# nerfstudio-project/gsplat

Measured on AMD Instinct MI355X. Metric: Mpixels/s fwd+bwd @1M Gaussians/1080p, higher is better.
Workload: dtype f32; 1 GPU; c3: 1M synthetic Gaussians, 1x1920x1080, SH deg 3, 16x16 tiles, fwd+bwd; gaussians_per_gpu=1000000, cameras_per_gpu=1, packed=False, parallelism=single

## Files before the change

gsplat_amd/csrc/projection.hip:

```cpp
#include "projmath.hpp"

namespace gsx {

struct ProjArgs {
    const float *means, *covars, *quats, *scales, *opacities, *viewmats, *Ks;
    uint32_t B, C, N, width, height;
    float eps2d, near_plane, far_plane, radius_clip;
    int camera_model;
    int calc_compensations;
    int32_t *radii;
    float *means2d, *depths, *conics, *compensations;
    int32_t *visible;
    const int64_t *row_offsets;
    int64_t nnz;
    int64_t *batch_ids, *camera_ids, *gaussian_ids;
    int32_t *indptr;
};

struct ProjOut {
    bool ok;
    int rx, ry;
    float mx, my, depth, ca, cb, cc, comp;
};

__device__ __forceinline__ void load_world_covar(const ProjArgs &a, uint32_t b, uint32_t g, float *S)
{
    if (a.covars) {
        const float *c = a.covars + ((size_t)b * a.N + g) * 6;
        S[0] = c[0]; S[1] = c[1]; S[2] = c[2];
        S[3] = c[1]; S[4] = c[3]; S[5] = c[4];
        S[6] = c[2]; S[7] = c[4]; S[8] = c[5];
    } else {
        const float *q = a.quats + ((size_t)b * a.N + g) * 4;
        const float *s = a.scales + ((size_t)b * a.N + g) * 3;
        float qn[4], Rq[9];
        quat_normalize(q, qn);
        quat_to_rotmat(qn, Rq);
        quat_scale_to_covar(Rq, s, false, S);
    }
}

__device__ __forceinline__ ProjOut project_one(const ProjArgs &a, uint32_t b, uint32_t c, uint32_t g, const float *p,
                                               float *world, bool *have_world)
{
    ProjOut o;
    o.ok = false;
    o.rx = o.ry = 0;
    o.mx = o.my = o.depth = o.ca = o.cb = o.cc = o.comp = 0.0f;
    const Cam cam  = load_cam(a.viewmats + ((size_t)b * a.C + c) * 16, a.Ks + ((size_t)b * a.C + c) * 9);
    float pc[3];
#pragma unroll
    for (int i = 0; i < 3; ++i) pc[i] = cam.R[3 * i] * p[0] + cam.R[3 * i + 1] * p[1] + cam.R[3 * i + 2] * p[2] + cam.t[i];
    if (pc[2] < a.near_plane || pc[2] > a.far_plane) return o;

    float RS[9], Sc[9];
    if (!*have_world) {
        load_world_covar(a, b, g, world);
        *have_world = true;
    }
    const float *S = world;
    mm3(cam.R, S, RS);
    mm3_nt(RS, cam.R, Sc);

    const Proj2D pr = project_camera(a.camera_model, cam, a.width, a.height, pc, Sc);
    const float det_orig = pr.a * pr.d - pr.b * pr.b;
    const float ca = pr.a + a.eps2d, cd = pr.d + a.eps2d;
    const float det_blur = ca * cd - pr.b * pr.b;
    if (det_blur <= 0.0f) return o;
    const float comp = sqrtf(fmaxf(kMinCompensation * kMinCompensation, det_orig / det_blur));

    float extend = kGaussianExtend;
    if (a.opacities) {
        float opacity = a.opacities[(size_t)b * a.N + g];
        if (a.calc_compensations) opacity *= comp;
        if (opacity < kAlphaThreshold) return o;
        extend = fminf(kGaussianExtend, sqrtf(2.0f * det_logf(opacity * 255.0f)));
    }
    const float rx = ceilf(extend * sqrtf(ca)), ry = ceilf(extend * sqrtf(cd));
    if (rx <= a.radius_clip && ry <= a.radius_clip) return o;
    if (pr.mx + rx <= 0.0f || pr.mx - rx >= (float)a.width || pr.my + ry <= 0.0f || pr.my - ry >= (float)a.height) return o;

    const float inv_det = 1.0f / det_blur;
    o.ok = true;
    o.rx = (int)rx; o.ry = (int)ry;
    o.mx = pr.mx; o.my = pr.my; o.depth = pc[2];
    o.ca = cd * inv_det; o.cb = -pr.b * inv_det; o.cc = ca * inv_det;
    o.comp = comp;
    return o;
}

__device__ __forceinline__ ProjOut project_one(const ProjArgs &a, uint32_t b, uint32_t c, uint32_t g)
{
    float world[9];
    bool have_world = false;
    return project_one(a, b, c, g, a.means + ((size_t)b * a.N + g) * 3, world, &have_world);
}

__global__ void __launch_bounds__(256) project_fwd_kernel(const ProjArgs a)
{
    const int64_t idx   = (int64_t)blockIdx.x * blockDim.x + threadIdx.x;
    const int64_t count = (int64_t)a.B * a.C * a.N;
    if (idx >= count) return;
    const uint32_t g = (uint32_t)(idx % a.N), c = (uint32_t)((idx / a.N) % a.C), b = (uint32_t)(idx / ((int64_t)a.N * a.C));
    const ProjOut o  = project_one(a, b, c, g);
    a.radii[2 * idx]       = o.rx;
    a.radii[2 * idx + 1]   = o.ry;
    a.means2d[2 * idx]     = o.mx;
    a.means2d[2 * idx + 1] = o.my;
    a.depths[idx]          = o.depth;
    a.conics[3 * idx]      = o.ca;
    a.conics[3 * idx + 1]  = o.cb;
    a.conics[3 * idx + 2]  = o.cc;
    if (a.compensations) a.compensations[idx] = o.comp;
}

__global__ void __launch_bounds__(256) project_fwd_gaussian_major_kernel(const ProjArgs a)
{
    const int64_t bg = (int64_t)blockIdx.x * blockDim.x + threadIdx.x;
    if (bg >= (int64_t)a.B * a.N) return;
    const uint32_t b = (uint32_t)(bg / a.N), g = (uint32_t)(bg % a.N);
    const float *pm = a.means + (size_t)bg * 3;
    const float p[3] = {pm[0], pm[1], pm[2]};
    float world[9];
    bool have_world = false;
    for (uint32_t c = 0; c < a.C; ++c) {
        const ProjOut o   = project_one(a, b, c, g, p, world, &have_world);
        const int64_t idx = ((int64_t)b * a.C + c) * a.N + g;
        a.radii[2 * idx]       = o.rx;
        a.radii[2 * idx + 1]   = o.ry;
        a.means2d[2 * idx]     = o.mx;
        a.means2d[2 * idx + 1] = o.my;
        a.depths[idx]          = o.depth;
        a.conics[3 * idx]      = o.ca;
        a.conics[3 * idx + 1]  = o.cb;
        a.conics[3 * idx + 2]  = o.cc;
        if (a.compensations) a.compensations[idx] = o.comp;
    }
}

__global__ void __launch_bounds__(256) project_count_kernel(const ProjArgs a)
{
    const int64_t idx   = (int64_t)blockIdx.x * blockDim.x + threadIdx.x;
    const int64_t count = (int64_t)a.B * a.C * a.N;
    if (idx >= count) return;
    const uint32_t g = (uint32_t)(idx % a.N), c = (uint32_t)((idx / a.N) % a.C), b = (uint32_t)(idx / ((int64_t)a.N * a.C));
    a.visible[idx]   = project_one(a, b, c, g).ok ? 1 : 0;
}

__global__ void __launch_bounds__(256) project_write_kernel(const ProjArgs a)
{
    const int64_t idx   = (int64_t)blockIdx.x * blockDim.x + threadIdx.x;
    const int64_t count = (int64_t)a.B * a.C * a.N;
    if (idx > count) return;
    if (idx % a.N == 0) {
        const int64_t img = idx / a.N;
        a.indptr[img]     = (int32_t)(idx == 0 ? 0 : a.row_offsets[idx - 1]);
    }
    if (idx == count) return;
    const int64_t row  = idx == 0 ? 0 : a.row_offsets[idx - 1];
    const int64_t next = a.row_offsets[idx];
    if (next == row) return;
    const uint32_t g = (uint32_t)(idx % a.N), c = (uint32_t)((idx / a.N) % a.C), b = (uint32_t)(idx / ((int64_t)a.N * a.C));
    const ProjOut o  = project_one(a, b, c, g);
    a.batch_ids[row]       = b;
    a.camera_ids[row]      = c;
    a.gaussian_ids[row]    = g;
    a.radii[2 * row]       = o.rx;
    a.radii[2 * row + 1]   = o.ry;
    a.means2d[2 * row]     = o.mx;
    a.means2d[2 * row + 1] = o.my;
    a.depths[row]          = o.depth;
    a.conics[3 * row]      = o.ca;
    a.conics[3 * row + 1]  = o.cb;
    a.conics[3 * row + 2]  = o.cc;
    if (a.compensations) a.compensations[row] = o.comp;
}

struct PackedBlocks {
    int32_t *block_counts;
    const int32_t *block_offsets;
};

__global__ void __launch_bounds__(256) project_count_blocks_kernel(const ProjArgs a, PackedBlocks pb)
{
    __shared__ int32_t s_n[4];
    const int64_t idx   = (int64_t)blockIdx.x * blockDim.x + threadIdx.x;
    const int64_t count = (int64_t)a.B * a.C * a.N;
    bool ok = false;
    if (idx < count) {
        const uint32_t g = (uint32_t)(idx % a.N), c = (uint32_t)((idx / a.N) % a.C), b = (uint32_t)(idx / ((int64_t)a.N * a.C));
        ok = project_one(a, b, c, g).ok;
    }
    const uint64_t m = __builtin_amdgcn_ballot_w64(ok);
    if ((threadIdx.x & 63u) == 0) s_n[threadIdx.x >> 6] = (int32_t)__popcll(m);
    __syncthreads();
    if (threadIdx.x == 0) pb.block_counts[blockIdx.x] = s_n[0] + s_n[1] + s_n[2] + s_n[3];
}

__global__ void __launch_bounds__(1024) packed_block_scan_kernel(const int32_t *counts, uint32_t n_blocks, int32_t *offsets,
                                                                int64_t *nnz_device, int64_t *nnz_host)
{
    __shared__ int64_t s_part[16];
    const int64_t total = block_scan_i32_1024(counts, offsets, n_blocks, s_part, nullptr);
    if (threadIdx.x == 0) {
        if (nnz_device) *nnz_device = total;
        if (nnz_host) {
            __threadfence_system();
            *nnz_host = total;
        }
    }
}

__global__ void __launch_bounds__(256) project_write_blocks_kernel(const ProjArgs a, PackedBlocks pb)
{
    __shared__ int32_t s_n[4];
    const int64_t idx   = (int64_t)blockIdx.x * blockDim.x + threadIdx.x;
    const int64_t count = (int64_t)a.B * a.C * a.N;
    const uint32_t lane = threadIdx.x & 63u, wave = threadIdx.x >> 6;
    uint32_t b = 0, c = 0, g = 0;
    ProjOut o;
    o.ok = false;
    if (idx < count) {
        g = (uint32_t)(idx % a.N); c = (uint32_t)((idx / a.N) % a.C); b = (uint32_t)(idx / ((int64_t)a.N * a.C));
        o = project_one(a, b, c, g);
    }
    const uint64_t m = __builtin_amdgcn_ballot_w64(o.ok);
    if (lane == 0) s_n[wave] = (int32_t)__popcll(m);
    __syncthreads();
    int32_t before = pb.block_offsets[blockIdx.x];
    for (uint32_t w = 0; w < wave; ++w) before += s_n[w];
    const int64_t row = (int64_t)before + (int64_t)__popcll(m & ((lane == 0) ? 0ull : (~0ull >> (64 - lane))));
    if (idx <= count && idx % a.N == 0) a.indptr[idx / a.N] = (int32_t)row;
    if (!o.ok) return;
    a.batch_ids[row]       = b;
    a.camera_ids[row]      = c;
    a.gaussian_ids[row]    = g;
    a.radii[2 * row]       = o.rx;
    a.radii[2 * row + 1]   = o.ry;
    a.means2d[2 * row]     = o.mx;
    a.means2d[2 * row + 1] = o.my;
    a.depths[row]          = o.depth;
    a.conics[3 * row]      = o.ca;
    a.conics[3 * row + 1]  = o.cb;
    a.conics[3 * row + 2]  = o.cc;
    if (a.compensations) a.compensations[row] = o.comp;
}

struct ProjBwdArgs {
    const float *means, *covars, *quats, *scales, *viewmats, *Ks;
    uint32_t B, C, N, width, height;
    float eps2d;
    int camera_model;
    const int32_t *radii;
    const float *conics, *compensations;
    const float *v_means2d, *v_depths, *v_conics, *v_compensations;
    uint32_t m2_stride, con_stride;
    int64_t nnz;
    const int64_t *batch_ids, *camera_ids, *gaussian_ids;
    const int32_t *row_map;
    int rows_out;
    float *v_means, *v_covars, *v_quats, *v_scales, *v_viewmats;
    const float *v_view_opacities;
    uint32_t opac_stride;
    float *v_opacities;
};

__device__ __forceinline__ void pair_vjp(const ProjBwdArgs &a, const Cam &cam, const float *p, const float *S,
                                         int64_t row, float *v_p, float *v_S, float *v_R, float *v_t, bool want_pose)
{
    const float ca = a.conics[3 * row], cb = a.conics[3 * row + 1], cc = a.conics[3 * row + 2];
    const float *vcon = a.v_conics + (size_t)a.con_stride * row;
    const float va = vcon[0], vb = 0.5f * vcon[1], vc = vcon[2];
    const float t00 = va * ca + vb * cb, t01 = va * cb + vb * cc;
    const float t10 = vb * ca + vc * cb, t11 = vb * cb + vc * cc;
    float g00 = -(ca * t00 + cb * t10);
    float g01 = -(ca * t01 + cb * t11);
    float g11 = -(cb * t01 + cc * t11);
    if (a.v_compensations) {
        const float comp = a.compensations[row], v_comp = a.v_compensations[row];
        const float detP = ca * cc - cb * cb;
        const float vsq  = v_comp * 0.5f / (comp + 1e-6f);
        const float omc  = 1.0f - comp * comp;
        g00 += vsq * (omc * ca - a.eps2d * detP);
        g01 += vsq * (omc * cb);
        g11 += vsq * (omc * cc - a.eps2d * detP);
    }
    float pc[3];
#pragma unroll
    for (int i = 0; i < 3; ++i) pc[i] = cam.R[3 * i] * p[0] + cam.R[3 * i + 1] * p[1] + cam.R[3 * i + 2] * p[2] + cam.t[i];
    float RS[9], Sc[9];
    mm3(cam.R, S, RS);
    mm3_nt(RS, cam.R, Sc);

    float v_pc[3] = {0.f, 0.f, 0.f}, v_Sc[9];
#pragma unroll
    for (int i = 0; i < 9; ++i) v_Sc[i] = 0.0f;
    const float *vm2 = a.v_means2d + (size_t)a.m2_stride * row;
    project_camera_vjp(a.camera_model, cam, a.width, a.height, pc, Sc, g00, g01, g11, vm2[0], vm2[1], v_pc, v_Sc);
    if (a.v_depths) v_pc[2] += a.v_depths[row];

#pragma unroll
    for (int j = 0; j < 3; ++j) v_p[j] += cam.R[j] * v_pc[0] + cam.R[3 + j] * v_pc[1] + cam.R[6 + j] * v_pc[2];
    float tmp[9], add[9];
    mm3_tn(cam.R, v_Sc, tmp);
    mm3(tmp, cam.R, add);
#pragma unroll
    for (int i = 0; i < 9; ++i) v_S[i] += add[i];
    if (want_pose) {
        float A1[9], A2[9];
        mm3(v_Sc, RS, A1);
        float v_ScT[9];
#pragma unroll
        for (int i = 0; i < 3; ++i)
#pragma unroll
            for (int j = 0; j < 3; ++j) v_ScT[3 * i + j] = v_Sc[3 * j + i];
        mm3(v_ScT, RS, A2);
#pragma unroll
        for (int i = 0; i < 3; ++i) {
#pragma unroll
            for (int j = 0; j < 3; ++j) v_R[3 * i + j] += v_pc[i] * p[j] + A1[3 * i + j] + A2[3 * i + j];
            v_t[i] += v_pc[i];
        }
    }
}

template <bool ATOMIC>
__device__ __forceinline__ void store_gaussian_grads(const ProjBwdArgs &a, uint32_t b, uint32_t g, size_t out,
                                                     const float *v_p, const float *v_S)
{
    const size_t bg = (size_t)b * a.N + g;
    auto put = [](float *dst, float v) {
        if (ATOMIC) atomic_add_f32(dst, v);
        else *dst = v;
    };
    if (a.v_means)
        for (int i = 0; i < 3; ++i) put(a.v_means + out * 3 + i, v_p[i]);
    if (a.covars) {
        if (a.v_covars) {
            put(a.v_covars + out * 6 + 0, v_S[0]);
            put(a.v_covars + out * 6 + 1, v_S[1] + v_S[3]);
            put(a.v_covars + out * 6 + 2, v_S[2] + v_S[6]);
            put(a.v_covars + out * 6 + 3, v_S[4]);
            put(a.v_covars + out * 6 + 4, v_S[5] + v_S[7]);
            put(a.v_covars + out * 6 + 5, v_S[8]);
        }
    } else {
        const float *q = a.quats + bg * 4;
        const float *s = a.scales + bg * 3;
        float qn[4], Rq[9], v_q[4] = {0.f, 0.f, 0.f, 0.f}, v_s[3] = {0.f, 0.f, 0.f};
        const float inv = quat_normalize(q, qn);
        quat_to_rotmat(qn, Rq);
        quat_scale_to_covar_vjp(qn, inv, Rq, s, v_S, v_q, v_s);
        if (a.v_quats)
            for (int i = 0; i < 4; ++i) put(a.v_quats + out * 4 + i, v_q[i]);
        if (a.v_scales)
            for (int i = 0; i < 3; ++i) put(a.v_scales + out * 3 + i, v_s[i]);
    }
}

__device__ __forceinline__ void reduce_pose_grads(float *v_viewmat , const float *v_R, const float *v_t)
{
    const uint32_t lane = threadIdx.x & 63u;
    float mine = 0.0f;
#pragma unroll
    for (int j = 0; j < 3; ++j) {
        const float r = wave_sum4_scatter(v_R[3 * j], v_R[3 * j + 1], v_R[3 * j + 2], v_t[j]);
        if ((int)(lane & 15u) == j) mine = r;
    }
    const int row = (int)(lane & 15u), col = (int)(lane >> 4);
    if (row < 3) atomic_add_f32(v_viewmat + 4 * row + col, mine);
}

#ifndef GSX_PROJ_BWD_WAVES
#define GSX_PROJ_BWD_WAVES 4
#endif
template <bool POSE>
__global__ void __launch_bounds__(256)
#if GSX_PROJ_BWD_WAVES
__attribute__((amdgpu_waves_per_eu(GSX_PROJ_BWD_WAVES)))
#endif
project_bwd_kernel(const ProjBwdArgs a)
{
    const int64_t idx = (int64_t)blockIdx.x * blockDim.x + threadIdx.x;
    const bool live   = idx < (int64_t)a.B * a.N;
    const uint32_t b = live ? (uint32_t)(idx / a.N) : 0, g = live ? (uint32_t)(idx % a.N) : 0;
    float p[3] = {0.f, 0.f, 0.f}, S[9];
    ProjArgs fa{};
    fa.covars = a.covars; fa.quats = a.quats; fa.scales = a.scales; fa.N = a.N;
    if (live) {
        const float *pm = a.means + ((size_t)b * a.N + g) * 3;
        p[0] = pm[0]; p[1] = pm[1]; p[2] = pm[2];
        load_world_covar(fa, b, g, S);
    }
    float v_p[3] = {0.f, 0.f, 0.f}, v_S[9];
#pragma unroll
    for (int i = 0; i < 9; ++i) v_S[i] = 0.0f;

    for (uint32_t c = 0; c < a.C; ++c) {
        float v_R[9], v_t[3] = {0.f, 0.f, 0.f};
#pragma unroll
        for (int i = 0; i < 9; ++i) v_R[i] = 0.0f;
        if (live) {
            int64_t row = ((int64_t)b * a.C + c) * a.N + g;
            bool visible;
            if (a.row_map) {
                row     = a.row_map[row];
                visible = row >= 0;
            } else {
                visible = a.radii[2 * row] > 0 && a.radii[2 * row + 1] > 0;
            }
            if (visible) {
                const Cam cam = load_cam(a.viewmats + ((size_t)b * a.C + c) * 16, a.Ks + ((size_t)b * a.C + c) * 9);
                pair_vjp(a, cam, p, S, row, v_p, v_S, v_R, v_t, POSE);
            }
        }
        if (POSE) {
            const uint32_t b_lo = __builtin_amdgcn_readfirstlane(b);
            uint32_t b_hi       = b_lo;
            {
                int m = wave_max_i32(live ? (int)b : (int)b_lo);
                b_hi  = (uint32_t)m;
            }
            for (uint32_t bb = b_lo; bb <= b_hi; ++bb) {
                float r[9], t[3];
                const bool sel = live && (b == bb);
#pragma unroll
                for (int i = 0; i < 9; ++i) r[i] = sel ? v_R[i] : 0.0f;
#pragma unroll
                for (int i = 0; i < 3; ++i) t[i] = sel ? v_t[i] : 0.0f;
                reduce_pose_grads(a.v_viewmats + ((size_t)bb * a.C + c) * 16, r, t);
            }
        }
    }
    if (live) store_gaussian_grads<false>(a, b, g, (size_t)b * a.N + g, v_p, v_S);
    if (live && a.v_opacities) {
        float v_o = 0.0f;
        for (uint32_t c = 0; c < a.C; ++c) {
            int64_t row = ((int64_t)b * a.C + c) * a.N + g;
            if (a.row_map) {
                row = a.row_map[row];
                if (row < 0) continue;
            }
            v_o += a.v_view_opacities[(size_t)row * a.opac_stride];
        }
        a.v_opacities[(size_t)b * a.N + g] = v_o;
    }
}

template <bool POSE, bool UNIQUE>
__global__ void __launch_bounds__(256) project_packed_bwd_kernel(const ProjBwdArgs a)
{
    const int64_t row = (int64_t)blockIdx.x * blockDim.x + threadIdx.x;
    const bool live   = row < a.nnz;
    uint32_t b = 0, c = 0, g = 0;
    float v_p[3] = {0.f, 0.f, 0.f}, v_S[9], v_R[9], v_t[3] = {0.f, 0.f, 0.f};
#pragma unroll
    for (int i = 0; i < 9; ++i) v_S[i] = v_R[i] = 0.0f;
    if (live) {
        b = (uint32_t)a.batch_ids[row]; c = (uint32_t)a.camera_ids[row]; g = (uint32_t)a.gaussian_ids[row];
        ProjArgs fa{};
        fa.covars = a.covars; fa.quats = a.quats; fa.scales = a.scales; fa.N = a.N;
        float S[9];
        load_world_covar(fa, b, g, S);
        const float *pm = a.means + ((size_t)b * a.N + g) * 3;
        const float p[3] = {pm[0], pm[1], pm[2]};
        const Cam cam = load_cam(a.viewmats + ((size_t)b * a.C + c) * 16, a.Ks + ((size_t)b * a.C + c) * 9);
        pair_vjp(a, cam, p, S, row, v_p, v_S, v_R, v_t, POSE);
        store_gaussian_grads<!UNIQUE>(a, b, g, a.rows_out ? (size_t)row : (size_t)b * a.N + g, v_p, v_S);
        if (a.v_opacities) {
            const float v_o = a.v_view_opacities[(size_t)row * a.opac_stride];
            if (UNIQUE) a.v_opacities[(size_t)b * a.N + g] = v_o;
            else atomic_add_f32(a.v_opacities + (size_t)b * a.N + g, v_o);
        }
    }
    if (POSE) {
        const int img  = live ? (int)(b * a.C + c) : -1;
        const int i_hi = wave_max_i32(img);
        int i_lo       = wave_max_i32(live ? -img : -2147483647);
        i_lo           = -i_lo;
        if (i_hi >= 0) {
            for (int im = i_lo; im <= i_hi; ++im) {
                float r[9], t[3];
                const bool sel = live && img == im;
                if (__builtin_amdgcn_ballot_w64(sel) == 0ull) continue;
#pragma unroll
                for (int i = 0; i < 9; ++i) r[i] = sel ? v_R[i] : 0.0f;
#pragma unroll
                for (int i = 0; i < 3; ++i) t[i] = sel ? v_t[i] : 0.0f;
                reduce_pose_grads(a.v_viewmats + (size_t)im * 16, r, t);
            }
        }
    }
}

__device__ __forceinline__ void store_sym(float *dst, const float *M, bool triu)
{
    if (triu) {
        dst[0] = M[0]; dst[1] = M[1]; dst[2] = M[2]; dst[3] = M[4]; dst[4] = M[5]; dst[5] = M[8];
    } else {
#pragma unroll
        for (int i = 0; i < 9; ++i) dst[i] = M[i];
    }
}

__global__ void __launch_bounds__(256) qs2c_fwd_kernel(const float *quats, const float *scales, int64_t n, int triu,
                                                       float *covars, float *precis)
{
    const int64_t i = (int64_t)blockIdx.x * blockDim.x + threadIdx.x;
    if (i >= n) return;
    float qn[4], Rq[9], M[9];
    quat_normalize(quats + 4 * i, qn);
    quat_to_rotmat(qn, Rq);
    const int stride = triu ? 6 : 9;
    if (covars) {
        quat_scale_to_covar(Rq, scales + 3 * i, false, M);
        store_sym(covars + stride * i, M, triu);
    }
    if (precis) {
        quat_scale_to_covar(Rq, scales + 3 * i, true, M);
        store_sym(precis + stride * i, M, triu);
    }
}

__device__ __forceinline__ void load_grad_sym(const float *src, bool triu, float *G)
{
    if (triu) {
        G[0] = src[0]; G[1] = 0.5f * src[1]; G[2] = 0.5f * src[2];
        G[3] = 0.5f * src[1]; G[4] = src[3]; G[5] = 0.5f * src[4];
        G[6] = 0.5f * src[2]; G[7] = 0.5f * src[4]; G[8] = src[5];
    } else {
#pragma unroll
        for (int i = 0; i < 9; ++i) G[i] = src[i];
    }
}

__global__ void __launch_bounds__(256) qs2c_bwd_kernel(const float *quats, const float *scales, int64_t n, int triu,
                                                       const float *v_covars, const float *v_precis, float *v_quats,
                                                       float *v_scales)
{
    const int64_t i = (int64_t)blockIdx.x * blockDim.x + threadIdx.x;
    if (i >= n) return;
    float qn[4], Rq[9], G[9], v_q[4] = {0.f, 0.f, 0.f, 0.f}, v_s[3] = {0.f, 0.f, 0.f};
    const float inv = quat_normalize(quats + 4 * i, qn);
    quat_to_rotmat(qn, Rq);
    const int stride = triu ? 6 : 9;
    if (v_covars) {
        load_grad_sym(v_covars + stride * i, triu, G);
        quat_scale_to_covar_vjp(qn, inv, Rq, scales + 3 * i, G, v_q, v_s);
    }
    if (v_precis) {
        load_grad_sym(v_precis + stride * i, triu, G);
        quat_scale_to_preci_vjp(qn, inv, Rq, scales + 3 * i, G, v_q, v_s);
    }
#pragma unroll
    for (int k = 0; k < 4; ++k) v_quats[4 * i + k] = v_q[k];
#pragma unroll
    for (int k = 0; k < 3; ++k) v_scales[3 * i + k] = v_s[k];
}

__global__ void __launch_bounds__(256) proj_simple_fwd_kernel(const float *means, const float *covars, const float *Ks,
                                                              int64_t rows, uint32_t N, uint32_t W, uint32_t H, int model,
                                                              float *means2d, float *covars2d)
{
    const int64_t idx = (int64_t)blockIdx.x * blockDim.x + threadIdx.x;
    if (idx >= rows) return;
    const float *K = Ks + (idx / N) * 9;
    Cam cam{};
    cam.fx = K[0]; cam.cx = K[2]; cam.fy = K[4]; cam.cy = K[5];
    const Proj2D pr = project_camera(model, cam, W, H, means + idx * 3, covars + idx * 9);
    means2d[2 * idx] = pr.mx; means2d[2 * idx + 1] = pr.my;
    covars2d[4 * idx] = pr.a; covars2d[4 * idx + 1] = pr.b; covars2d[4 * idx + 2] = pr.b; covars2d[4 * idx + 3] = pr.d;
}

__global__ void __launch_bounds__(256) proj_simple_bwd_kernel(const float *means, const float *covars, const float *Ks,
                                                              int64_t rows, uint32_t N, uint32_t W, uint32_t H, int model,
                                                              const float *v_means2d, const float *v_covars2d,
                                                              float *v_means, float *v_covars)
{
    const int64_t idx = (int64_t)blockIdx.x * blockDim.x + threadIdx.x;
    if (idx >= rows) return;
    const float *K = Ks + (idx / N) * 9;
    Cam cam{};
    cam.fx = K[0]; cam.cx = K[2]; cam.fy = K[4]; cam.cy = K[5];
    const float *p = means + idx * 3, *Sc = covars + idx * 9, *V = v_covars2d + idx * 4;
    float v_p[3] = {0.f, 0.f, 0.f}, v_Sc[9];
#pragma unroll
    for (int i = 0; i < 9; ++i) v_Sc[i] = 0.0f;
    const float g01 = 0.5f * (V[1] + V[2]), an = 0.5f * (V[1] - V[2]);
    project_camera_vjp(model, cam, W, H, p, Sc, V[0], g01, V[3], v_means2d[2 * idx], v_means2d[2 * idx + 1], v_p, v_Sc);
    const Proj2D pr = project_camera(model, cam, W, H, p, Sc);
#pragma unroll
    for (int i = 0; i < 3; ++i)
#pragma unroll
        for (int j = 0; j < 3; ++j) v_Sc[3 * i + j] += an * (pr.J[i] * pr.J[3 + j] - pr.J[3 + i] * pr.J[j]);
#pragma unroll
    for (int i = 0; i < 3; ++i) v_means[idx * 3 + i] = v_p[i];
#pragma unroll
    for (int i = 0; i < 9; ++i) v_covars[idx * 9 + i] = v_Sc[i];
}

__global__ void __launch_bounds__(256) packed_row_map_kernel(const int64_t *batch_ids, const int64_t *camera_ids,
                                                             const int64_t *gaussian_ids, int64_t nnz, uint32_t C, uint32_t N,
                                                             int32_t *row_map)
{
    const int64_t r = (int64_t)blockIdx.x * blockDim.x + threadIdx.x;
    if (r >= nnz) return;
    row_map[(batch_ids[r] * C + camera_ids[r]) * (int64_t)N + gaussian_ids[r]] = (int32_t)r;
}

static int check_proj_common(const char *fn, const float *means, const float *covars, const float *quats,
                             const float *scales, const float *viewmats, const float *Ks, int camera_model)
{
    GSX_REQUIRE(means && viewmats && Ks, "%s: null means/viewmats/Ks", fn);
    GSX_REQUIRE(covars || (quats && scales), "%s: need covars or (quats and scales)", fn);
    GSX_REQUIRE(camera_model == GSX_CAMERA_PINHOLE || camera_model == GSX_CAMERA_ORTHO || camera_model == GSX_CAMERA_FISHEYE,
                "%s: unsupported camera model %d (pinhole/ortho/fisheye only)", fn, camera_model);
    return GSX_OK;
}

}

using namespace gsx;


static ProjArgs proj_args(const float *means, const float *covars, const float *quats, const float *scales,
                          const float *opacities, const float *viewmats, const float *Ks, uint32_t B, uint32_t C, uint32_t N,
                          uint32_t width, uint32_t height, float eps2d, float near_plane, float far_plane, float radius_clip,
                          int camera_model, int calc_compensations)
{
    ProjArgs a{};
    a.means = means; a.covars = covars; a.quats = quats; a.scales = scales; a.opacities = opacities;
    a.viewmats = viewmats; a.Ks = Ks; a.B = B; a.C = C; a.N = N; a.width = width; a.height = height;
    a.eps2d = eps2d; a.near_plane = near_plane; a.far_plane = far_plane; a.radius_clip = radius_clip;
    a.camera_model = camera_model; a.calc_compensations = calc_compensations;
    return a;
}
static void proj_rows(ProjArgs &a, int32_t *radii, float *means2d, float *depths, float *conics, float *compensations)
{
    a.radii = radii; a.means2d = means2d; a.depths = depths; a.conics = conics; a.compensations = compensations;
    a.calc_compensations = compensations != nullptr;
}

extern "C" int gsx_project_ewa_fwd(const float *means, const float *covars, const float *quats, const float *scales,
                                   const float *opacities, const float *viewmats, const float *Ks, uint32_t B,
                                   uint32_t C, uint32_t N, uint32_t width, uint32_t height, float eps2d,
                                   float near_plane, float far_plane, float radius_clip, int camera_model,
                                   int32_t *radii, float *means2d, float *depths, float *conics, float *compensations,
                                   void *stream)
{
    const int64_t count = (int64_t)B * C * N;
    if (count == 0) return GSX_OK;
    int rc = check_proj_common("gsx_project_ewa_fwd", means, covars, quats, scales, viewmats, Ks, camera_model);
    if (rc != GSX_OK) return rc;
    GSX_REQUIRE(radii && means2d && depths && conics, "gsx_project_ewa_fwd: null output");
    ProjArgs a = proj_args(means, covars, quats, scales, opacities, viewmats, Ks, B, C, N, width, height, eps2d, near_plane,
                           far_plane, radius_clip, camera_model, 0);
    proj_rows(a, radii, means2d, depths, conics, compensations);
    if (C > 1)
        project_fwd_gaussian_major_kernel<<<dim3((uint32_t)ceil_div((int64_t)B * N, 256)), dim3(256), 0, (hipStream_t)stream>>>(a);
    else
        project_fwd_kernel<<<dim3((uint32_t)ceil_div(count, 256)), dim3(256), 0, (hipStream_t)stream>>>(a);
    return check_launch("project_ewa_fwd");
}

extern "C" int gsx_project_ewa_packed_count(const float *means, const float *covars, const float *quats,
                                            const float *scales, const float *opacities, const float *viewmats,
                                            const float *Ks, uint32_t B, uint32_t C, uint32_t N, uint32_t width,
                                            uint32_t height, float eps2d, float near_plane, float far_plane,
                                            float radius_clip, int camera_model, int calc_compensations,
                                            int32_t *visible, void *stream)
{
    const int64_t count = (int64_t)B * C * N;
    if (count == 0) return GSX_OK;
    int rc = check_proj_common("gsx_project_ewa_packed_count", means, covars, quats, scales, viewmats, Ks, camera_model);
    if (rc != GSX_OK) return rc;
    GSX_REQUIRE(visible, "gsx_project_ewa_packed_count: null output");
    ProjArgs a = proj_args(means, covars, quats, scales, opacities, viewmats, Ks, B, C, N, width, height, eps2d, near_plane,
                           far_plane, radius_clip, camera_model, calc_compensations);
    a.visible = visible;
    project_count_kernel<<<dim3((uint32_t)ceil_div(count, 256)), dim3(256), 0, (hipStream_t)stream>>>(a);
    return check_launch("project_ewa_packed_count");
}

extern "C" int gsx_project_ewa_packed_write(const float *means, const float *covars, const float *quats,
                                            const float *scales, const float *opacities, const float *viewmats,
                                            const float *Ks, uint32_t B, uint32_t C, uint32_t N, uint32_t width,
                                            uint32_t height, float eps2d, float near_plane, float far_plane,
                                            float radius_clip, int camera_model, const int64_t *row_offsets,
                                            int64_t nnz, int64_t *batch_ids, int64_t *camera_ids,
                                            int64_t *gaussian_ids, int32_t *indptr, int32_t *radii, float *means2d,
                                            float *depths, float *conics, float *compensations, void *stream)
{
    const int64_t count = (int64_t)B * C * N;
    GSX_REQUIRE(indptr, "gsx_project_ewa_packed_write: null indptr");
    if (count == 0) {
        if (hipMemsetAsync(indptr, 0, ((size_t)B * C + 1) * sizeof(int32_t), (hipStream_t)stream) != hipSuccess) {
            set_last_error("gsx_project_ewa_packed_write: memset failed");
            return GSX_ERR_LAUNCH;
        }
        return GSX_OK;
    }
    int rc = check_proj_common("gsx_project_ewa_packed_write", means, covars, quats, scales, viewmats, Ks, camera_model);
    if (rc != GSX_OK) return rc;
    GSX_REQUIRE(row_offsets, "gsx_project_ewa_packed_write: null row_offsets");
    GSX_REQUIRE(nnz == 0 || (batch_ids && camera_ids && gaussian_ids && radii && means2d && depths && conics),
                "gsx_project_ewa_packed_write: null output");
    ProjArgs a = proj_args(means, covars, quats, scales, opacities, viewmats, Ks, B, C, N, width, height, eps2d, near_plane,
                           far_plane, radius_clip, camera_model, 0);
    proj_rows(a, radii, means2d, depths, conics, compensations);
    a.row_offsets = row_offsets; a.nnz = nnz; a.batch_ids = batch_ids; a.camera_ids = camera_ids;
    a.gaussian_ids = gaussian_ids; a.indptr = indptr;
    project_write_kernel<<<dim3((uint32_t)ceil_div(count + 1, 256)), dim3(256), 0, (hipStream_t)stream>>>(a);
    return check_launch("project_ewa_packed_write");
}

extern "C" int64_t gsx_project_packed_blocks(int64_t pairs) { return (pairs + 1 + 255) / 256; }

extern "C" int gsx_project_ewa_packed_count_blocks(const float *means, const float *covars, const float *quats,
                                                   const float *scales, const float *opacities, const float *viewmats,
                                                   const float *Ks, uint32_t B, uint32_t C, uint32_t N, uint32_t width,
                                                   uint32_t height, float eps2d, float near_plane, float far_plane,
                                                   float radius_clip, int camera_model, int calc_compensations,
                                                   int32_t *block_counts, int32_t *block_offsets, int64_t *nnz_device,
                                                   int64_t *nnz_host, void *stream)
{
    const int64_t count = (int64_t)B * C * N;
    GSX_REQUIRE(count < (1ll << 31) - 256, "gsx_project_ewa_packed_count_blocks: %lld (image, Gaussian) pairs exceed int32 offsets",
                (long long)count);
    GSX_REQUIRE(block_counts && block_offsets, "gsx_project_ewa_packed_count_blocks: null block buffer");
    if (count > 0) {
        int rc = check_proj_common("gsx_project_ewa_packed_count_blocks", means, covars, quats, scales, viewmats, Ks, camera_model);
        if (rc != GSX_OK) return rc;
    }
    const ProjArgs a = proj_args(means, covars, quats, scales, opacities, viewmats, Ks, B, C, N, width, height, eps2d, near_plane,
                                 far_plane, radius_clip, camera_model, calc_compensations);
    PackedBlocks pb{block_counts, block_offsets};
    const uint32_t n_blocks = (uint32_t)gsx_project_packed_blocks(count);
    project_count_blocks_kernel<<<dim3(n_blocks), dim3(256), 0, (hipStream_t)stream>>>(a, pb);
    packed_block_scan_kernel<<<dim3(1), dim3(1024), 0, (hipStream_t)stream>>>(block_counts, n_blocks, block_offsets, nnz_device,
                                                                            nnz_host);
    return check_launch("project_ewa_packed_count_blocks");
}

extern "C" int gsx_project_ewa_packed_write_blocks(const float *means, const float *covars, const float *quats,
                                                   const float *scales, const float *opacities, const float *viewmats,
                                                   const float *Ks, uint32_t B, uint32_t C, uint32_t N, uint32_t width,
                                                   uint32_t height, float eps2d, float near_plane, float far_plane,
                                                   float radius_clip, int camera_model, const int32_t *block_offsets,
                                                   int64_t *batch_ids, int64_t *camera_ids, int64_t *gaussian_ids,
                                                   int32_t *indptr, int32_t *radii, float *means2d, float *depths,
                                                   float *conics, float *compensations, void *stream)
{
    const int64_t count = (int64_t)B * C * N;
    GSX_REQUIRE(indptr && block_offsets, "gsx_project_ewa_packed_write_blocks: null indptr / block offsets");
    GSX_REQUIRE(count < (1ll << 31) - 256, "gsx_project_ewa_packed_write_blocks: too many (image, Gaussian) pairs");
    if (count == 0) {
        if (hipMemsetAsync(indptr, 0, ((size_t)B * C + 1) * sizeof(int32_t), (hipStream_t)stream) != hipSuccess) {
            set_last_error("gsx_project_ewa_packed_write_blocks: memset failed");
            return GSX_ERR_LAUNCH;
        }
        return GSX_OK;
    }
    if (count > 0) {
        int rc = check_proj_common("gsx_project_ewa_packed_write_blocks", means, covars, quats, scales, viewmats, Ks, camera_model);
        if (rc != GSX_OK) return rc;
        GSX_REQUIRE(batch_ids && camera_ids && gaussian_ids && radii && means2d && depths && conics,
                    "gsx_project_ewa_packed_write_blocks: null output");
    }
    ProjArgs a = proj_args(means, covars, quats, scales, opacities, viewmats, Ks, B, C, N, width, height, eps2d, near_plane,
                           far_plane, radius_clip, camera_model, 0);
    proj_rows(a, radii, means2d, depths, conics, compensations);
    a.batch_ids = batch_ids; a.camera_ids = camera_ids; a.gaussian_ids = gaussian_ids; a.indptr = indptr;
    PackedBlocks pb{nullptr, block_offsets};
    project_write_blocks_kernel<<<dim3((uint32_t)gsx_project_packed_blocks(count)), dim3(256), 0, (hipStream_t)stream>>>(a, pb);
    return check_launch("project_ewa_packed_write_blocks");
}

static ProjBwdArgs proj_bwd_args(const float *means, const float *covars, const float *quats, const float *scales,
                                 const float *viewmats, const float *Ks, uint32_t B, uint32_t C, uint32_t N, uint32_t width,
                                 uint32_t height, float eps2d, int camera_model, const float *conics,
                                 const float *compensations, const float *v_means2d, uint32_t m2_stride, const float *v_depths,
                                 const float *v_conics, uint32_t con_stride, const float *v_compensations, float *v_means,
                                 float *v_covars, float *v_quats, float *v_scales, float *v_viewmats)
{
    ProjBwdArgs a{};
    a.m2_stride = m2_stride; a.con_stride = con_stride;
    a.means = means; a.covars = covars; a.quats = quats; a.scales = scales; a.viewmats = viewmats; a.Ks = Ks;
    a.B = B; a.C = C; a.N = N; a.width = width; a.height = height; a.eps2d = eps2d; a.camera_model = camera_model;
    a.conics = conics; a.compensations = compensations; a.v_means2d = v_means2d; a.v_depths = v_depths;
    a.v_conics = v_conics; a.v_compensations = (compensations && v_compensations) ? v_compensations : nullptr;
    a.v_means = v_means; a.v_covars = v_covars; a.v_quats = v_quats; a.v_scales = v_scales; a.v_viewmats = v_viewmats;
    return a;
}

static int check_proj_bwd(const char *fn, const ProjBwdArgs &a, bool packed)
{
    int rc = check_proj_common(fn, a.means, a.covars, a.quats, a.scales, a.viewmats, a.Ks, a.camera_model);
    if (rc != GSX_OK) return rc;
    GSX_REQUIRE((packed ? a.batch_ids && a.camera_ids && a.gaussian_ids : a.radii != nullptr) && a.conics && a.v_means2d
                && a.v_conics, "%s: null input", fn);
    GSX_REQUIRE(a.m2_stride >= 2 && a.con_stride >= 3, "%s: row strides must be >= 2 / >= 3", fn);
    return GSX_OK;
}

static int zero_v_opacities(const char *fn, const ProjBwdArgs &a, hipStream_t s)
{
    if (hipMemsetAsync(a.v_opacities, 0, (size_t)a.B * a.N * sizeof(float), s) != hipSuccess) {
        set_last_error("%s: memset failed", fn);
        return GSX_ERR_LAUNCH;
    }
    return GSX_OK;
}

static int launch_project_bwd(const char *fn, const ProjBwdArgs &a, hipStream_t s)
{
    const dim3 grid((uint32_t)ceil_div((int64_t)a.B * a.N, 256)), block(256);
    if (a.v_viewmats) project_bwd_kernel<true><<<grid, block, 0, s>>>(a);
    else project_bwd_kernel<false><<<grid, block, 0, s>>>(a);
    return check_launch(fn + 4);
}

static int project_bwd(const char *fn, const ProjBwdArgs &a, bool opac, hipStream_t s)
{
    const int64_t count = (int64_t)a.B * a.N;
    if (count == 0 || (!opac && a.C == 0)) return GSX_OK;
    if (opac) {
        GSX_REQUIRE(a.v_opacities, "%s: null v_opacities", fn);
        if (a.C == 0) return zero_v_opacities(fn, a, s);
        GSX_REQUIRE(a.v_view_opacities && a.opac_stride >= 1, "%s: null opacity cotangent", fn);
    }
    int rc = check_proj_bwd(fn, a, false);
    if (rc != GSX_OK) return rc;
    return launch_project_bwd(fn, a, s);
}

static int project_packed_bwd(const char *fn, const ProjBwdArgs &a, bool opac, hipStream_t s)
{
    if (opac) {
        if ((int64_t)a.B * a.N == 0) return GSX_OK;
        GSX_REQUIRE(a.v_opacities, "%s: null v_opacities", fn);
        if (a.nnz <= 0) return zero_v_opacities(fn, a, s);
        GSX_REQUIRE(a.v_view_opacities && a.opac_stride >= 1, "%s: null opacity cotangent", fn);
    } else if (a.nnz <= 0) return GSX_OK;
    int rc = check_proj_bwd(fn, a, true);
    if (rc != GSX_OK) return rc;
    if (a.row_map) return launch_project_bwd(fn, a, s);
    const dim3 grid((uint32_t)ceil_div(a.nnz, 256)), block(256);
    const bool unique = (uint64_t)a.B * a.C == 1;
    if (a.v_viewmats) {
        if (unique) project_packed_bwd_kernel<true, true><<<grid, block, 0, s>>>(a);
        else project_packed_bwd_kernel<true, false><<<grid, block, 0, s>>>(a);
    } else {
        if (unique) project_packed_bwd_kernel<false, true><<<grid, block, 0, s>>>(a);
        else project_packed_bwd_kernel<false, false><<<grid, block, 0, s>>>(a);
    }
    return check_launch(fn + 4);
}

extern "C" int gsx_project_ewa_bwd(const float *means, const float *covars, const float *quats, const float *scales,
                                   const float *viewmats, const float *Ks, uint32_t B, uint32_t C, uint32_t N,
                                   uint32_t width, uint32_t height, float eps2d, int camera_model,
                                   const int32_t *radii, const float *conics, const float *compensations,
                                   const float *v_means2d, uint32_t v_means2d_stride, const float *v_depths,
                                   const float *v_conics, uint32_t v_conics_stride,
                                   const float *v_compensations, float *v_means, float *v_covars, float *v_quats,
                                   float *v_scales, float *v_viewmats, void *stream)
{
    ProjBwdArgs a = proj_bwd_args(means, covars, quats, scales, viewmats, Ks, B, C, N, width, height, eps2d, camera_model, conics,
                                  compensations, v_means2d, v_means2d_stride, v_depths, v_conics, v_conics_stride,
                                  v_compensations, v_means, v_covars, v_quats, v_scales, v_viewmats);
    a.radii = radii;
    return project_bwd("gsx_project_ewa_bwd", a, false, (hipStream_t)stream);
}

extern "C" int gsx_project_ewa_bwd_opac(const float *means, const float *covars, const float *quats, const float *scales,
                                        const float *viewmats, const float *Ks, uint32_t B, uint32_t C, uint32_t N,
                                        uint32_t width, uint32_t height, float eps2d, int camera_model,
                                        const int32_t *radii, const float *conics, const float *compensations,
                                        const float *v_means2d, uint32_t v_means2d_stride, const float *v_depths,
                                        const float *v_conics, uint32_t v_conics_stride, const float *v_compensations,
                                        const float *v_view_opacities, uint32_t v_view_opacities_stride, float *v_means,
                                        float *v_covars, float *v_quats, float *v_scales, float *v_viewmats,
                                        float *v_opacities, void *stream)
{
    ProjBwdArgs a = proj_bwd_args(means, covars, quats, scales, viewmats, Ks, B, C, N, width, height, eps2d, camera_model, conics,
                                  compensations, v_means2d, v_means2d_stride, v_depths, v_conics, v_conics_stride,
                                  v_compensations, v_means, v_covars, v_quats, v_scales, v_viewmats);
    a.radii = radii;
    a.v_view_opacities = v_view_opacities; a.opac_stride = v_view_opacities_stride; a.v_opacities = v_opacities;
    return project_bwd("gsx_project_ewa_bwd_opac", a, true, (hipStream_t)stream);
}

extern "C" int gsx_project_ewa_packed_bwd(const float *means, const float *covars, const float *quats,
                                          const float *scales, const float *viewmats, const float *Ks, uint32_t B,
                                          uint32_t C, uint32_t N, uint32_t width, uint32_t height, float eps2d,
                                          int camera_model, int64_t nnz, const int64_t *batch_ids,
                                          const int64_t *camera_ids, const int64_t *gaussian_ids, const float *conics,
                                          const float *compensations, const float *v_means2d,
                                          uint32_t v_means2d_stride, const float *v_depths, const float *v_conics,
                                          uint32_t v_conics_stride, const float *v_compensations,
                                          const int32_t *row_map, float *v_means, float *v_covars, float *v_quats,
                                          float *v_scales, float *v_viewmats, void *stream)
{
    ProjBwdArgs a = proj_bwd_args(means, covars, quats, scales, viewmats, Ks, B, C, N, width, height, eps2d, camera_model, conics,
                                  compensations, v_means2d, v_means2d_stride, v_depths, v_conics, v_conics_stride,
                                  v_compensations, v_means, v_covars, v_quats, v_scales, v_viewmats);
    a.nnz = nnz; a.batch_ids = batch_ids; a.camera_ids = camera_ids; a.gaussian_ids = gaussian_ids; a.row_map = row_map;
    return project_packed_bwd("gsx_project_ewa_packed_bwd", a, false, (hipStream_t)stream);
}

extern "C" int gsx_project_ewa_packed_bwd_opac(const float *means, const float *covars, const float *quats,
                                               const float *scales, const float *viewmats, const float *Ks, uint32_t B,
                                               uint32_t C, uint32_t N, uint32_t width, uint32_t height, float eps2d,
                                               int camera_model, int64_t nnz, const int64_t *batch_ids,
                                               const int64_t *camera_ids, const int64_t *gaussian_ids, const float *conics,
                                               const float *compensations, const float *v_means2d,
                                               uint32_t v_means2d_stride, const float *v_depths, const float *v_conics,
                                               uint32_t v_conics_stride, const float *v_compensations,
                                               const float *v_view_opacities, uint32_t v_view_opacities_stride,
                                               const int32_t *row_map, float *v_means, float *v_covars, float *v_quats,
                                               float *v_scales, float *v_viewmats, float *v_opacities, void *stream)
{
    ProjBwdArgs a = proj_bwd_args(means, covars, quats, scales, viewmats, Ks, B, C, N, width, height, eps2d, camera_model, conics,
                                  compensations, v_means2d, v_means2d_stride, v_depths, v_conics, v_conics_stride,
                                  v_compensations, v_means, v_covars, v_quats, v_scales, v_viewmats);
    a.nnz = nnz; a.batch_ids = batch_ids; a.camera_ids = camera_ids; a.gaussian_ids = gaussian_ids; a.row_map = row_map;
    a.v_view_opacities = v_view_opacities; a.opac_stride = v_view_opacities_stride; a.v_opacities = v_opacities;
    return project_packed_bwd("gsx_project_ewa_packed_bwd_opac", a, true, (hipStream_t)stream);
}

extern "C" int gsx_project_ewa_packed_bwd_rows(const float *means, const float *covars, const float *quats,
                                               const float *scales, const float *viewmats, const float *Ks, uint32_t B,
                                               uint32_t C, uint32_t N, uint32_t width, uint32_t height, float eps2d,
                                               int camera_model, int64_t nnz, const int64_t *batch_ids,
                                               const int64_t *camera_ids, const int64_t *gaussian_ids,
                                               const float *conics, const float *compensations, const float *v_means2d,
                                               uint32_t v_means2d_stride, const float *v_depths, const float *v_conics,
                                               uint32_t v_conics_stride, const float *v_compensations,
                                               float *v_means_rows, float *v_covars_rows, float *v_quats_rows,
                                               float *v_scales_rows, float *v_viewmats, void *stream)
{
    if (nnz <= 0) return GSX_OK;
    ProjBwdArgs a = proj_bwd_args(means, covars, quats, scales, viewmats, Ks, B, C, N, width, height, eps2d, camera_model, conics,
                                  compensations, v_means2d, v_means2d_stride, v_depths, v_conics, v_conics_stride,
                                  v_compensations, v_means_rows, v_covars_rows, v_quats_rows, v_scales_rows, v_viewmats);
    a.nnz = nnz; a.batch_ids = batch_ids; a.camera_ids = camera_ids; a.gaussian_ids = gaussian_ids;
    a.rows_out = 1;
    int rc = check_proj_bwd("gsx_project_ewa_packed_bwd_rows", a, true);
    if (rc != GSX_OK) return rc;
    const dim3 grid((uint32_t)ceil_div(nnz, 256)), block(256);
    if (v_viewmats) project_packed_bwd_kernel<true, true><<<grid, block, 0, (hipStream_t)stream>>>(a);
    else project_packed_bwd_kernel<false, true><<<grid, block, 0, (hipStream_t)stream>>>(a);
    return check_launch("project_ewa_packed_bwd_rows");
}

extern "C" int gsx_quat_scale_to_covar_fwd(const float *quats, const float *scales, int64_t n, int triu,
                                           float *covars, float *precis, void *stream)
{
    if (n <= 0) return GSX_OK;
    GSX_REQUIRE(quats && scales, "gsx_quat_scale_to_covar_fwd: null input");
    qs2c_fwd_kernel<<<dim3((uint32_t)ceil_div(n, 256)), dim3(256), 0, (hipStream_t)stream>>>(quats, scales, n, triu,
                                                                                           covars, precis);
    return check_launch("quat_scale_to_covar_fwd");
}

extern "C" int gsx_quat_scale_to_covar_bwd(const float *quats, const float *scales, int64_t n, int triu,
                                           const float *v_covars, const float *v_precis, float *v_quats,
                                           float *v_scales, void *stream)
{
    if (n <= 0) return GSX_OK;
    GSX_REQUIRE(quats && scales && v_quats && v_scales, "gsx_quat_scale_to_covar_bwd: null pointer");
    qs2c_bwd_kernel<<<dim3((uint32_t)ceil_div(n, 256)), dim3(256), 0, (hipStream_t)stream>>>(
        quats, scales, n, triu, v_covars, v_precis, v_quats, v_scales);
    return check_launch("quat_scale_to_covar_bwd");
}

extern "C" int gsx_project_simple_fwd(const float *means, const float *covars, const float *Ks, int64_t rows,
                                      uint32_t n_per_camera, uint32_t width, uint32_t height, int camera_model,
                                      float *means2d, float *covars2d, void *stream)
{
    if (rows == 0) return GSX_OK;
    GSX_REQUIRE(means && covars && Ks && means2d && covars2d && n_per_camera > 0, "gsx_project_simple_fwd: bad argument");
    proj_simple_fwd_kernel<<<dim3((uint32_t)ceil_div(rows, 256)), dim3(256), 0, (hipStream_t)stream>>>(
        means, covars, Ks, rows, n_per_camera, width, height, camera_model, means2d, covars2d);
    return check_launch("project_simple_fwd");
}

extern "C" int gsx_project_simple_bwd(const float *means, const float *covars, const float *Ks, int64_t rows,
                                      uint32_t n_per_camera, uint32_t width, uint32_t height, int camera_model,
                                      const float *v_means2d, const float *v_covars2d, float *v_means, float *v_covars,
                                      void *stream)
{
    if (rows == 0) return GSX_OK;
    GSX_REQUIRE(means && covars && Ks && v_means2d && v_covars2d && v_means && v_covars && n_per_camera > 0,
                "gsx_project_simple_bwd: bad argument");
    proj_simple_bwd_kernel<<<dim3((uint32_t)ceil_div(rows, 256)), dim3(256), 0, (hipStream_t)stream>>>(
        means, covars, Ks, rows, n_per_camera, width, height, camera_model, v_means2d, v_covars2d, v_means, v_covars);
    return check_launch("project_simple_bwd");
}

extern "C" int gsx_packed_row_map(const int64_t *batch_ids, const int64_t *camera_ids, const int64_t *gaussian_ids,
                                  int64_t nnz, uint32_t B, uint32_t C, uint32_t N, int32_t *row_map, void *stream)
{
    const int64_t total = (int64_t)B * C * N;
    if (total == 0) return GSX_OK;
    GSX_REQUIRE(row_map, "gsx_packed_row_map: null output");
    GSX_REQUIRE(nnz >= 0 && nnz < (1ll << 31), "gsx_packed_row_map: nnz out of range");
    hipStream_t s = (hipStream_t)stream;
    if (hipMemsetAsync(row_map, 0xFF, (size_t)total * sizeof(int32_t), s) != hipSuccess) {
        set_last_error("gsx_packed_row_map: memset failed");
        return GSX_ERR_LAUNCH;
    }
    if (nnz == 0) return GSX_OK;
    GSX_REQUIRE(batch_ids && camera_ids && gaussian_ids, "gsx_packed_row_map: null ids");
    packed_row_map_kernel<<<dim3((uint32_t)ceil_div(nnz, 256)), dim3(256), 0, s>>>(batch_ids, camera_ids, gaussian_ids, nnz, C,
                                                                                  N, row_map);
    return check_launch("packed_row_map");
}
```

Baseline: 2450 Mpixels/s.

## Compact live Gaussians per block in projection backward and skip dead waves

The projection backward kernel first scans each Gaussian's per-camera cotangents and radii to decide whether it has any nonzero gradient. It then compacts live threads to the front of the workgroup through a shared-memory permutation, so whole waves made only of dead Gaussians just write zero gradients and exit. Camera loads are also made wave-uniform through constant address space, and the kernel is specialised on row_map. The cost is an extra pre-pass that reads the per-row inputs twice, plus scattered memory access caused by the permutation.

```diff
diff --git a/gsplat_amd/csrc/projection.hip b/gsplat_amd/csrc/projection.hip
--- a/gsplat_amd/csrc/projection.hip
+++ b/gsplat_amd/csrc/projection.hip
@@ -265,19 +265,48 @@
     float *v_opacities;
 };
 
+struct PairRow {
+    float ca, cb, cc;
+    float va, vb2, vc;
+    float comp, v_comp;
+    float vm0, vm1, v_d;
+    __device__ __forceinline__ bool live() const
+    {
+        return (vm0 != 0.0f) | (vm1 != 0.0f) | (va != 0.0f) | (vb2 != 0.0f) | (vc != 0.0f) | (v_d != 0.0f) | (v_comp != 0.0f);
+    }
+};
+
+__device__ __forceinline__ PairRow load_pair_row(const ProjBwdArgs &a, int64_t row)
+{
+    PairRow r;
+    const float *con  = a.conics + 3 * row;
+    const float *vcon = a.v_conics + (size_t)a.con_stride * row;
+    const float *vm2  = a.v_means2d + (size_t)a.m2_stride * row;
+    const float *pcomp = a.v_compensations ? a.compensations + row : con;
+    const float *pvcmp = a.v_compensations ? a.v_compensations + row : con;
+    const float *pvd   = a.v_depths ? a.v_depths + row : con;
+    r.ca = con[0]; r.cb = con[1]; r.cc = con[2];
+    r.va = vcon[0]; r.vb2 = vcon[1]; r.vc = vcon[2];
+    r.vm0 = vm2[0]; r.vm1 = vm2[1];
+    const float comp = *pcomp, v_comp = *pvcmp, v_d = *pvd;
+    r.comp = comp;
+    r.v_comp = a.v_compensations ? v_comp : 0.0f;
+    r.v_d = a.v_depths ? v_d : 0.0f;
+    return r;
+}
+
 __device__ __forceinline__ void pair_vjp(const ProjBwdArgs &a, const Cam &cam, const float *p, const float *S,
-                                         int64_t row, float *v_p, float *v_S, float *v_R, float *v_t, bool want_pose)
-{
-    const float ca = a.conics[3 * row], cb = a.conics[3 * row + 1], cc = a.conics[3 * row + 2];
-    const float *vcon = a.v_conics + (size_t)a.con_stride * row;
-    const float va = vcon[0], vb = 0.5f * vcon[1], vc = vcon[2];
+                                         const PairRow &r, float *v_p, float *v_S, float *v_R, float *v_t, bool want_pose)
+{
+    const float ca = r.ca, cb = r.cb, cc = r.cc;
+    const float va = r.va, vb = 0.5f * r.vb2, vc = r.vc;
     const float t00 = va * ca + vb * cb, t01 = va * cb + vb * cc;
     const float t10 = vb * ca + vc * cb, t11 = vb * cb + vc * cc;
     float g00 = -(ca * t00 + cb * t10);
     float g01 = -(ca * t01 + cb * t11);
     float g11 = -(cb * t01 + cc * t11);
     if (a.v_compensations) {
-        const float comp = a.compensations[row], v_comp = a.v_compensations[row];
+        const float comp = r.comp, v_comp = r.v_comp;
         const float detP = ca * cc - cb * cb;
         const float vsq  = v_comp * 0.5f / (comp + 1e-6f);
         const float omc  = 1.0f - comp * comp;
@@ -295,9 +324,8 @@
     float v_pc[3] = {0.f, 0.f, 0.f}, v_Sc[9];
 #pragma unroll
     for (int i = 0; i < 9; ++i) v_Sc[i] = 0.0f;
-    const float *vm2 = a.v_means2d + (size_t)a.m2_stride * row;
-    project_camera_vjp(a.camera_model, cam, a.width, a.height, pc, Sc, g00, g01, g11, vm2[0], vm2[1], v_pc, v_Sc);
-    if (a.v_depths) v_pc[2] += a.v_depths[row];
+    project_camera_vjp(a.camera_model, cam, a.width, a.height, pc, Sc, g00, g01, g11, r.vm0, r.vm1, v_pc, v_Sc);
+    if (a.v_depths) v_pc[2] += r.v_d;
 
 #pragma unroll
     for (int j = 0; j < 3; ++j) v_p[j] += cam.R[j] * v_pc[0] + cam.R[3 + j] * v_pc[1] + cam.R[6 + j] * v_pc[2];
@@ -371,80 +399,180 @@
     if (row < 3) atomic_add_f32(v_viewmat + 4 * row + col, mine);
 }
 
+template <bool MAPPED>
+__device__ __forceinline__ void row_radii(const ProjBwdArgs &a, int64_t &row, int32_t &rx, int32_t &ry)
+{
+    if (MAPPED) {
+        const int32_t r = a.row_map[row];
+        rx = ry = r >= 0;
+        row     = r >= 0 ? r : 0;
+    } else {
+        rx = a.radii[2 * row];
+        ry = a.radii[2 * row + 1];
+    }
+}
+
+__device__ __forceinline__ void split_bg(const ProjBwdArgs &a, int64_t idx, uint32_t &b, uint32_t &g)
+{
+    if (a.B == 1) {
+        b = 0;
+        g = (uint32_t)idx;
+    } else {
+        b = (uint32_t)(idx / a.N);
+        g = (uint32_t)(idx % a.N);
+    }
+}
+
+__device__ __forceinline__ void store_zero_grads(const ProjBwdArgs &a, size_t out)
+{
+    if (a.v_means)
+        for (int i = 0; i < 3; ++i) a.v_means[out * 3 + i] = 0.0f;
+    if (a.covars) {
+        if (a.v_covars)
+            for (int i = 0; i < 6; ++i) a.v_covars[out * 6 + i] = 0.0f;
+    } else {
+        if (a.v_quats)
+            for (int i = 0; i < 4; ++i) a.v_quats[out * 4 + i] = 0.0f;
+        if (a.v_scales)
+            for (int i = 0; i < 3; ++i) a.v_scales[out * 3 + i] = 0.0f;
+    }
+}
+
+__device__ __forceinline__ Cam load_cam_uniform(const float *viewmat , const float *K )
+{
+    typedef const float __attribute__((address_space(4))) cfloat;
+    const cfloat *vm = (const cfloat *)(uintptr_t)viewmat;
+    const cfloat *k  = (const cfloat *)(uintptr_t)K;
+    Cam c;
+#pragma unroll
+    for (int i = 0; i < 3; ++i) {
+#pragma unroll
+        for (int j = 0; j < 3; ++j) c.R[3 * i + j] = vm[4 * i + j];
+        c.t[i] = vm[4 * i + 3];
+    }
+    c.fx = k[0]; c.cx = k[2]; c.fy = k[4]; c.cy = k[5];
+    return c;
+}
+
 #ifndef GSX_PROJ_BWD_WAVES
 #define GSX_PROJ_BWD_WAVES 4
 #endif
-template <bool POSE>
-__global__ void __launch_bounds__(256)
+#ifndef GSX_PROJ_BWD_THREADS
+#define GSX_PROJ_BWD_THREADS 256
+#endif
+constexpr uint32_t kProjBwdThreads = GSX_PROJ_BWD_THREADS;
+static_assert(kProjBwdThreads % 64 == 0 && kProjBwdThreads >= 64 && kProjBwdThreads <= 1024, "whole waves, one workgroup");
+
+template <bool POSE, bool MAPPED>
+__global__ void __launch_bounds__(kProjBwdThreads)
 #if GSX_PROJ_BWD_WAVES
 __attribute__((amdgpu_waves_per_eu(GSX_PROJ_BWD_WAVES)))
 #endif
 project_bwd_kernel(const ProjBwdArgs a)
 {
-    const int64_t idx = (int64_t)blockIdx.x * blockDim.x + threadIdx.x;
-    const bool live   = idx < (int64_t)a.B * a.N;
-    const uint32_t b = live ? (uint32_t)(idx / a.N) : 0, g = live ? (uint32_t)(idx % a.N) : 0;
-    float p[3] = {0.f, 0.f, 0.f}, S[9];
+    constexpr uint32_t NW = kProjBwdThreads / 64;
+    __shared__ uint32_t s_live[NW];
+    __shared__ uint16_t s_order[kProjBwdThreads];
+    const uint32_t t = threadIdx.x, lane = t & 63u, wave = t >> 6;
+    const int64_t total = (int64_t)a.B * a.N;
+    const int64_t base  = (int64_t)blockIdx.x * kProjBwdThreads;
+
+    bool alive = false;
+    {
+        const int64_t idx = base + t;
+        if (idx < total) {
+            uint32_t b, g;
+            split_bg(a, idx, b, g);
+            float v_o = 0.0f;
+            if (MAPPED) {
+                for (uint32_t c = 0; c < a.C; ++c) {
+                    const int64_t row = a.row_map[((int64_t)b * a.C + c) * a.N + g];
+                    if (row < 0) continue;
+                    const PairRow r = load_pair_row(a, row);
+                    if (a.v_opacities) v_o += a.v_view_opacities[(size_t)row * a.opac_stride];
+                    alive = alive | r.live();
+                }
+            } else {
+                for (uint32_t c = 0; c < a.C; ++c) {
+                    const int64_t row = ((int64_t)b * a.C + c) * a.N + g;
+                    const int32_t rx = a.radii[2 * row], ry = a.radii[2 * row + 1];
+                    const PairRow r = load_pair_row(a, row);
+                    if (a.v_opacities) v_o += a.v_view_opacities[(size_t)row * a.opac_stride];
+                    alive = alive | ((rx > 0) & (ry > 0) & r.live());
+                }
+            }
+            if (a.v_opacities) a.v_opacities[idx] = v_o;
+        }
+    }
+
+    const uint64_t m     = __builtin_amdgcn_ballot_w64(alive);
+    const uint32_t below = __builtin_amdgcn_mbcnt_hi((uint32_t)(m >> 32), __builtin_amdgcn_mbcnt_lo((uint32_t)m, 0u));
+    if (lane == 0) s_live[wave] = (uint32_t)__builtin_popcountll(m);
+    __syncthreads();
+    uint32_t n_live = 0, live_before = 0;
+#pragma unroll
+    for (uint32_t w = 0; w < NW; ++w) {
+        const uint32_t n = s_live[w];
+        n_live += n;
+        if (w < wave) live_before += n;
+    }
+    n_live = __builtin_amdgcn_readfirstlane(n_live);
+    s_order[alive ? live_before + below : kProjBwdThreads - 1u - ((wave * 64u - live_before) + (lane - below))] = (uint16_t)t;
+    __syncthreads();
+
+    const uint32_t local = s_order[t];
+    if ((t & ~63u) >= n_live) {
+        if (base + local < total) store_zero_grads(a, (size_t)(base + local));
+        return;
+    }
+    const bool work   = t < n_live;
+    const int64_t idx = work ? base + local : base;
+    uint32_t b, g;
+    split_bg(a, idx, b, g);
+
+    const float *pm = a.means + (size_t)idx * 3;
+    const float p[3] = {pm[0], pm[1], pm[2]};
+    int64_t row = (int64_t)b * a.C * a.N + g;
+    int32_t rx, ry;
+    row_radii<MAPPED>(a, row, rx, ry);
+    PairRow pr   = load_pair_row(a, row);
+    bool visible = (rx > 0) & (ry > 0);
+    float S[9];
     ProjArgs fa{};
     fa.covars = a.covars; fa.quats = a.quats; fa.scales = a.scales; fa.N = a.N;
-    if (live) {
-        const float *pm = a.means + ((size_t)b * a.N + g) * 3;
-        p[0] = pm[0]; p[1] = pm[1]; p[2] = pm[2];
-        load_world_covar(fa, b, g, S);
-    }
+    load_world_covar(fa, b, g, S);
+
     float v_p[3] = {0.f, 0.f, 0.f}, v_S[9];
 #pragma unroll
     for (int i = 0; i < 9; ++i) v_S[i] = 0.0f;
 
-    for (uint32_t c = 0; c < a.C; ++c) {
+    const uint32_t b_lo = __builtin_amdgcn_readfirstlane(b);
+    const uint32_t b_hi = (uint32_t)wave_max_i32(work ? (int)b : (int)b_lo);
+    for (uint32_t c = 0;;) {
         float v_R[9], v_t[3] = {0.f, 0.f, 0.f};
 #pragma unroll
         for (int i = 0; i < 9; ++i) v_R[i] = 0.0f;
-        if (live) {
-            int64_t row = ((int64_t)b * a.C + c) * a.N + g;
-            bool visible;
-            if (a.row_map) {
-                row     = a.row_map[row];
-                visible = row >= 0;
-            } else {
-                visible = a.radii[2 * row] > 0 && a.radii[2 * row + 1] > 0;
-            }
-            if (visible) {
-                const Cam cam = load_cam(a.viewmats + ((size_t)b * a.C + c) * 16, a.Ks + ((size_t)b * a.C + c) * 9);
-                pair_vjp(a, cam, p, S, row, v_p, v_S, v_R, v_t, POSE);
+        for (uint32_t bb = b_lo; bb <= b_hi; ++bb) {
+            const Cam cam  = load_cam_uniform(a.viewmats + ((size_t)bb * a.C + c) * 16, a.Ks + ((size_t)bb * a.C + c) * 9);
+            const bool sel = work && b == bb;
+            if (sel && visible) pair_vjp(a, cam, p, S, pr, v_p, v_S, v_R, v_t, POSE);
+            if (POSE) {
+                float r[9], tt[3];
+#pragma unroll
+                for (int i = 0; i < 9; ++i) r[i] = sel ? v_R[i] : 0.0f;
+#pragma unroll
+                for (int i = 0; i < 3; ++i) tt[i] = sel ? v_t[i] : 0.0f;
+                reduce_pose_grads(a.v_viewmats + ((size_t)bb * a.C + c) * 16, r, tt);
             }
         }
-        if (POSE) {
-            const uint32_t b_lo = __builtin_amdgcn_readfirstlane(b);
-            uint32_t b_hi       = b_lo;
-            {
-                int m = wave_max_i32(live ? (int)b : (int)b_lo);
-                b_hi  = (uint32_t)m;
-            }
-            for (uint32_t bb = b_lo; bb <= b_hi; ++bb) {
-                float r[9], t[3];
-                const bool sel = live && (b == bb);
-#pragma unroll
-                for (int i = 0; i < 9; ++i) r[i] = sel ? v_R[i] : 0.0f;
-#pragma unroll
-                for (int i = 0; i < 3; ++i) t[i] = sel ? v_t[i] : 0.0f;
-                reduce_pose_grads(a.v_viewmats + ((size_t)bb * a.C + c) * 16, r, t);
-            }
-        }
-    }
-    if (live) store_gaussian_grads<false>(a, b, g, (size_t)b * a.N + g, v_p, v_S);
-    if (live && a.v_opacities) {
-        float v_o = 0.0f;
-        for (uint32_t c = 0; c < a.C; ++c) {
-            int64_t row = ((int64_t)b * a.C + c) * a.N + g;
-            if (a.row_map) {
-                row = a.row_map[row];
-                if (row < 0) continue;
-            }
-            v_o += a.v_view_opacities[(size_t)row * a.opac_stride];
-        }
-        a.v_opacities[(size_t)b * a.N + g] = v_o;
-    }
+        if (++c == a.C) break;
+        row = ((int64_t)b * a.C + c) * a.N + g;
+        row_radii<MAPPED>(a, row, rx, ry);
+        pr      = load_pair_row(a, row);
+        visible = (rx > 0) & (ry > 0);
+    }
+    if (work) store_gaussian_grads<false>(a, b, g, (size_t)idx, v_p, v_S);
+    else if (base + local < total) store_zero_grads(a, (size_t)(base + local));
 }
 
 template <bool POSE, bool UNIQUE>
@@ -465,7 +593,7 @@
         const float *pm = a.means + ((size_t)b * a.N + g) * 3;
         const float p[3] = {pm[0], pm[1], pm[2]};
         const Cam cam = load_cam(a.viewmats + ((size_t)b * a.C + c) * 16, a.Ks + ((size_t)b * a.C + c) * 9);
-        pair_vjp(a, cam, p, S, row, v_p, v_S, v_R, v_t, POSE);
+        pair_vjp(a, cam, p, S, load_pair_row(a, row), v_p, v_S, v_R, v_t, POSE);
         store_gaussian_grads<!UNIQUE>(a, b, g, a.rows_out ? (size_t)row : (size_t)b * a.N + g, v_p, v_S);
         if (a.v_opacities) {
             const float v_o = a.v_view_opacities[(size_t)row * a.opac_stride];
@@ -814,9 +942,14 @@
 
 static int launch_project_bwd(const char *fn, const ProjBwdArgs &a, hipStream_t s)
 {
-    const dim3 grid((uint32_t)ceil_div((int64_t)a.B * a.N, 256)), block(256);
-    if (a.v_viewmats) project_bwd_kernel<true><<<grid, block, 0, s>>>(a);
-    else project_bwd_kernel<false><<<grid, block, 0, s>>>(a);
+    const dim3 grid((uint32_t)ceil_div((int64_t)a.B * a.N, kProjBwdThreads)), block(kProjBwdThreads);
+    if (a.row_map) {
+        if (a.v_viewmats) project_bwd_kernel<true, true><<<grid, block, 0, s>>>(a);
+        else project_bwd_kernel<false, true><<<grid, block, 0, s>>>(a);
+    } else {
+        if (a.v_viewmats) project_bwd_kernel<true, false><<<grid, block, 0, s>>>(a);
+        else project_bwd_kernel<false, false><<<grid, block, 0, s>>>(a);
+    }
     return check_launch(fn + 4);
 }
 
```

Result: no change. 2465 Mpixels/s, median of 6 (+0.6%).
